# ruc-aimc-lab/GeoFormer

Measured on NVIDIA B200. Metric: pairs_per_sec_640x480, higher is better.
Workload: dtype tf32 / fp16 tensor-core operands with fp32 accumulation (fp32 residual stream, fp16 intermediates), split-fp16 similarity, f16 backbone activations

## Files before the change

geoformer_b200/_lib.py:

```python
from __future__ import annotations

import ctypes
import os
from ctypes import c_char_p, c_float, c_int, c_int64, c_void_p

HERE = os.path.dirname(os.path.abspath(__file__))
LIB_PATH = os.path.join(HERE, "libgeoformer_sm100.so")

P, I, L, F = c_void_p, c_int, c_int64, c_float

SIGNATURES = {
    "gf_abi_version": (I, []),
    "gf_last_error": (c_char_p, []),
    "gf_init": (I, [I]),
    "gf_launch_count": (L, []),
    "gf_linear_tf32": (I, [P, P, P, P, L, I, I, I, I, I, P, P, I, P, P, P, P, P]),
    "gf_linear_ref": (I, [P, P, P, P, L, I, I, I, I, I, P, P, I, P, P, P, P, P]),
    "gf_conv3x3_f16": (I, [P, P, P, P, P, I, I, I, I, I, I, I, P]),
    "gf_conv_f16": (I, [P, P, P, P, P, I, I, I, I, I, I, I, I, I, P]),
    "gf_stem_conv7x7_f16": (I, [P, P, P, P, I, I, I, P]),
    "gf_upsample_add_f16": (I, [P, P, P, I, I, I, I, I, I, P]),
    "gf_conv_ref": (I, [P, P, P, P, P, I, I, I, I, I, I, I, I, P]),
    "gf_upsample_add_ref": (I, [P, P, P, I, I, I, I, I, I, P]),
    "gf_add_posenc": (I, [P, P, P, I, L, I, P]),
    "gf_linattn_partial_floats": (L, [I, I, I, I]),
    "gf_linear_mixed": (I, [P, P, P, P, I, I, L, I, I, I, I, I, P, P, I, P, P, P, P, P]),
    "gf_fine_layer": (I, [P, P, P, P, P, P, P, P, L, P]),
    "gf_linattn_reduce_f16": (I, [P, I, P, I, I, I, I, I, P, P, P, P]),
    "gf_linattn_apply_f16": (I, [P, I, P, P, P, I, I, I, I, I, P]),
    "gf_linattn_window_f16": (I, [P, I, P, I, P, I, P, L, I, I, I, P]),
    "gf_linattn_reduce": (I, [P, I, P, I, I, I, I, I, P, P, P, P]),
    "gf_linattn_apply": (I, [P, I, P, P, P, I, I, I, I, I, P]),
    "gf_linattn_window": (I, [P, I, P, I, P, I, P, L, I, I, I, P]),
    "gf_pack_split_f16": (I, [P, P, L, I, F, I, P]),
    "gf_similarity_f16x3": (I, [P, P, P, I, I, I, I, F, P]),
    "gf_similarity_ref": (I, [P, P, P, I, I, I, I, F, F, P]),
    "gf_dual_softmax_workspace_floats": (L, [I, I, I]),
    "gf_dual_softmax_stats": (I, [P, I, I, I, P, P, P, P, P, P]),
    "gf_dual_softmax_conf": (I, [P, I, I, I, P, P, P, P, P, P, P]),
    "gf_conf_row_col_max": (I, [P, I, I, I, P, P, P]),
    "gf_mnn_select": (I, [P, I, I, I, F, I, I, I, I, I, P, P, P, P, P]),
    "gf_coarse_match_fused_workspace_bytes": (L, [I, I, I]),
    "gf_coarse_match_fused": (I, [P, P, I, I, I, I, F, F, I, I, I, I, I, P, P, P, P]),
    "gf_coarse_match_fused_pass": (I, [P, P, I, I, I, I, F, P, I, P]),
    "gf_compact_coarse": (I, [P, P, I, I, I, I, F, P, P, P, P, P, P, P, P, L, P]),
    "gf_geo_window_table": (I, [P, P, I, I, I, I, I, I, I, I, P, P]),
    "gf_geo_self_attention": (I, [P, I, P, I, P, I, P, I, I, I, I, P, P, I, P]),
    "gf_gather_anchor_kv": (I, [P, I, P, I, I, I, I, I, P, P, I, I, P, P, P]),
    "gf_gather_anchor_kv_f16": (I, [P, I, P, I, P, I, I, I, I, I, P, P, I, I, P, P, P, P]),
    "gf_geo_self_attention_tc": (I, [P, I, P, P, P, I, I, I, I, I, P, P]),
    "gf_gather_anchor_kv_h16": (I, [P, I, P, I, I, I, I, I, P, P, I, I, P, P, P]),
    "gf_masked_softmax_rows": (I, [P, I, I, I, I, P, P]),
    "gf_gemm_tf32_batched": (I, [P, L, L, P, L, L, P, L, L, I, I, I, I, F, P]),
    "gf_geo_cross_attention": (I, [P, I, P, I, P, I, P, I, I, I, I, I, P, I, P]),
    "gf_geo_cross_attention_f16": (I, [P, I, P, I, P, I, P, I, I, I, I, I, P, I, P]),
    "gf_select_rows": (I, [P, P, P, I, L, I, P]),
    "gf_fine_gather": (I, [P, I, I, I, P, P, L, I, I, I, P, P]),
    "gf_fine_gather_f16": (I, [P, I, I, I, P, P, L, I, I, I, P, P]),
    "gf_fine_gather_f16_f16": (I, [P, I, I, I, P, P, L, I, I, I, P, P]),
    "gf_gather_rows": (I, [P, L, I, P, P, L, P, P]),
    "gf_fine_match": (I, [P, P, L, I, I, F, F, P, P, P, P, P, P]),
    "gf_resize_gray_u8": (I, [P, I, I, P, I, I, P]),
    "gf_ransac_workspace_bytes": (L, [I, I]),
    "gf_ransac_homography": (I, [P, P, P, P, L, I, I, F, ctypes.c_uint, I, I, I, I, I, P, P, P, P, P, P, P, P, P, P, P, I, P]),
    "gf_compact_fine": (I, [P, P, P, P, P, P, P, L, I, F, F, F, P, P, P, P, P, P]),
    "gf_mask_rows": (I, [P, I, L, L, L, L, P, P]),
    "gf_mask_fill_sim": (I, [P, I, I, I, P, P, F, P]),
}


class GeoFormerLibError(RuntimeError):
    pass


_lib = None
_initialised_devices = set()


def load() -> ctypes.CDLL:
    global _lib
    if _lib is not None:
        return _lib
    if not os.path.exists(LIB_PATH):
        raise GeoFormerLibError(
            f"{LIB_PATH} not found - build it with `python -m geoformer_b200.build` "
            "(there is no CPU or PyTorch fallback for the hot path)")
    lib = ctypes.CDLL(LIB_PATH)
    for name, (res, args) in SIGNATURES.items():
        fn = getattr(lib, name)
        fn.restype = res
        fn.argtypes = args
    if lib.gf_abi_version() != 1:
        raise GeoFormerLibError("ABI version mismatch")
    _lib = lib
    return lib


def init(device_index: int) -> None:
    lib = load()
    if device_index in _initialised_devices:
        return
    rc = lib.gf_init(int(device_index))
    if rc != 0:
        raise GeoFormerLibError(f"gf_init({device_index}) failed: {lib.gf_last_error().decode()} (rc={rc})")
    _initialised_devices.add(device_index)


def call(name: str, *args):
    lib = load()
    rc = getattr(lib, name)(*args)
    if rc != 0:
        raise GeoFormerLibError(f"{name} failed: {lib.gf_last_error().decode()} (rc={rc})")


def launch_count() -> int:
    return int(load().gf_launch_count())
```

geoformer_b200/csrc/geo_attention.cu:

```cuda
#include "common.cuh"

#include <atomic>
#include <cuda_fp16.h>

namespace gf {
extern std::atomic<int64_t> g_launches;

__global__ void geo_window_table_kernel(const float* __restrict__ hmat, const int* __restrict__ has_h, int n, int l,
                                        int w_src_c, int h_dst_px, int w_dst_px, int w_dst_c, int scale, int window,
                                        int* __restrict__ widx) {
  const int64_t idx = (int64_t)blockIdx.x * blockDim.x + threadIdx.x;
  if (idx >= (int64_t)n * l) return;
  const int b = (int)(idx / l);
  const int tok = (int)(idx - (int64_t)b * l);
  int* out = widx + idx * window * window;
  if (!has_h[b]) {
    for (int w = 0; w < window * window; ++w) out[w] = -1;
    return;
  }
  const float* H = hmat + b * 9;
  const float x = (float)((tok % w_src_c) * scale), y = (float)((tok / w_src_c) * scale);
  float wx = __fmaf_rn(H[2], 1.f, __fmaf_rn(H[1], y, __fmul_rn(H[0], x)));
  float wy = __fmaf_rn(H[5], 1.f, __fmaf_rn(H[4], y, __fmul_rn(H[3], x)));
  float wz = __fmaf_rn(H[8], 1.f, __fmaf_rn(H[7], y, __fmul_rn(H[6], x)));
  if (wz == 0.f) wz = 1e-6f;
  const float cx = __fdiv_rn(wx, wz), cy = __fdiv_rn(wy, wz);
  const int half = window / 2;
  for (int r = 0; r < window; ++r) {
    for (int c = 0; c < window; ++c) {
      const float kx = __fadd_rn(cx, (float)((c - half) * scale));
      const float ky = __fadd_rn(cy, (float)((r - half) * scale));
      const bool oob = (kx < 0.f) | (ky < 0.f) | (kx >= (float)w_dst_px) | (ky >= (float)h_dst_px) | !(kx == kx) | !(ky == ky);
      int t = -1;
      if (!oob) t = ((int)ky / scale) * w_dst_c + ((int)kx / scale);
      out[r * window + c] = t;
    }
  }
}

constexpr int kSA = 64;
constexpr int kSAPad = kSA + 4;

__global__ void __launch_bounds__(256)
geo_self_attention_kernel(const float* __restrict__ q, int ldq, const float* __restrict__ k, int ldk,
                          const float* __restrict__ v, int ldv, float* __restrict__ out, int l, int heads,
                          const int* __restrict__ anchor_idx, const int* __restrict__ anchor_cnt, int anchor_cap,
                          float softmax_scale) {
  extern __shared__ float sh[];
  float* Qs = sh;
  float* Kt = Qs + kSA * kSA;
  float* Vs = Kt + kSA * kSAPad;
  float* Ps = Vs + kSA * kSAPad;
  const int n = blockIdx.z, h = blockIdx.y, q0 = blockIdx.x * kSA;
  const int cnt = anchor_cnt[n];
  const int c = heads * kSA;
  const int tid = threadIdx.x, tx = tid & 15, ty = tid >> 4;
  if (cnt == 0) {
    for (int e = tid; e < kSA * kSA; e += 256) {
      const int r = e >> 6, d = e & 63;
      if (q0 + r < l) out[((int64_t)n * l + q0 + r) * c + h * kSA + d] = 0.f;
    }
    return;
  }
  for (int e = tid; e < kSA * kSA; e += 256) {
    const int r = e >> 6, d = e & 63;
    Qs[e] = (q0 + r < l) ? q[((int64_t)n * l + q0 + r) * ldq + h * kSA + d] : 0.f;
  }
  float m_run[4], l_run[4], o[4][4];
#pragma unroll
  for (int i = 0; i < 4; ++i) {
    m_run[i] = -INFINITY; l_run[i] = 0.f;
#pragma unroll
    for (int j = 0; j < 4; ++j) o[i][j] = 0.f;
  }
  const int* aidx = anchor_idx + (int64_t)n * anchor_cap;
  for (int k0 = 0; k0 < cnt; k0 += kSA) {
    __syncthreads();
    for (int e = tid; e < kSA * kSA; e += 256) {
      const int r = e >> 6, d = e & 63;
      float kv = 0.f, vv = 0.f;
      if (k0 + r < cnt) {
        const int64_t tok = (int64_t)n * l + aidx[k0 + r];
        kv = k[tok * ldk + h * kSA + d];
        vv = v[tok * ldv + h * kSA + d];
      }
// ... 11 lines not shown
      const float4 kk = *reinterpret_cast<const float4*>(&Kt[d * kSAPad + 4 * tx]);
#pragma unroll
      for (int i = 0; i < 4; ++i) {
        const float qv = Qs[(4 * ty + i) * kSA + d];
        s[i][0] = fmaf(qv, kk.x, s[i][0]); s[i][1] = fmaf(qv, kk.y, s[i][1]);
        s[i][2] = fmaf(qv, kk.z, s[i][2]); s[i][3] = fmaf(qv, kk.w, s[i][3]);
      }
    }
    float alpha[4];
#pragma unroll
    for (int i = 0; i < 4; ++i) {
      float mx = -INFINITY;
#pragma unroll
      for (int j = 0; j < 4; ++j) {
        s[i][j] = (k0 + 4 * tx + j < cnt) ? s[i][j] * softmax_scale : -INFINITY;
        mx = fmaxf(mx, s[i][j]);
      }
#pragma unroll
      for (int off = 8; off > 0; off >>= 1) mx = fmaxf(mx, __shfl_xor_sync(0xffffffffu, mx, off));
      const float m_new = fmaxf(m_run[i], mx);
      alpha[i] = expf(m_run[i] - m_new);
      float rs = 0.f;
#pragma unroll
      for (int j = 0; j < 4; ++j) { s[i][j] = expf(s[i][j] - m_new); rs += s[i][j]; }
#pragma unroll
      for (int off = 8; off > 0; off >>= 1) rs += __shfl_xor_sync(0xffffffffu, rs, off);
      l_run[i] = l_run[i] * alpha[i] + rs;
      m_run[i] = m_new;
      *reinterpret_cast<float4*>(&Ps[(4 * ty + i) * kSAPad + 4 * tx]) = make_float4(s[i][0], s[i][1], s[i][2], s[i][3]);
#pragma unroll
      for (int j = 0; j < 4; ++j) o[i][j] *= alpha[i];
    }
    __syncthreads();
#pragma unroll 8
    for (int kk = 0; kk < kSA; ++kk) {
      const float4 vv = *reinterpret_cast<const float4*>(&Vs[kk * kSAPad + 4 * tx]);
#pragma unroll
      for (int i = 0; i < 4; ++i) {
        const float pv = Ps[(4 * ty + i) * kSAPad + kk];
        o[i][0] = fmaf(pv, vv.x, o[i][0]); o[i][1] = fmaf(pv, vv.y, o[i][1]);
        o[i][2] = fmaf(pv, vv.z, o[i][2]); o[i][3] = fmaf(pv, vv.w, o[i][3]);
      }
    }
  }
#pragma unroll
  for (int i = 0; i < 4; ++i) {
    const int r = q0 + 4 * ty + i;
    if (r < l) {
      const float inv = 1.f / l_run[i];
      *reinterpret_cast<float4*>(&out[((int64_t)n * l + r) * c + h * kSA + 4 * tx]) =
          make_float4(o[i][0] * inv, o[i][1] * inv, o[i][2] * inv, o[i][3] * inv);
    }
  }
}

__device__ __forceinline__ void load8(const float* p, float (&v)[8]) {
  const float4 a = *reinterpret_cast<const float4*>(p), b = *reinterpret_cast<const float4*>(p + 4);
  v[0] = a.x; v[1] = a.y; v[2] = a.z; v[3] = a.w; v[4] = b.x; v[5] = b.y; v[6] = b.z; v[7] = b.w;
}
__device__ __forceinline__ void load8(const __half* p, float (&v)[8]) {
  const uint4 u = *reinterpret_cast<const uint4*>(p);
  const uint32_t w[4] = {u.x, u.y, u.z, u.w};
#pragma unroll
  for (int i = 0; i < 4; ++i) {
    const float2 f = __half22float2(*reinterpret_cast<const __half2*>(&w[i]));
    v[2 * i] = f.x; v[2 * i + 1] = f.y;
  }
}
__device__ __forceinline__ void store8(float* p, const float (&v)[8]) {
  *reinterpret_cast<float4*>(p) = make_float4(v[0], v[1], v[2], v[3]);
  *reinterpret_cast<float4*>(p + 4) = make_float4(v[4], v[5], v[6], v[7]);
}
__device__ __forceinline__ void store8(__half* p, const float (&v)[8]) {
  uint4 u;
  __half2 h;
  h = __floats2half2_rn(v[0], v[1]); u.x = *reinterpret_cast<uint32_t*>(&h);
  h = __floats2half2_rn(v[2], v[3]); u.y = *reinterpret_cast<uint32_t*>(&h);
  h = __floats2half2_rn(v[4], v[5]); u.z = *reinterpret_cast<uint32_t*>(&h);
  h = __floats2half2_rn(v[6], v[7]); u.w = *reinterpret_cast<uint32_t*>(&h);
  *reinterpret_cast<uint4*>(p) = u;
}

template <typename T>
__global__ void geo_cross_attention_kernel(const T* __restrict__ q, int ldq, const T* __restrict__ kp, int ldk,
                                           const T* __restrict__ vp, int ldv, T* __restrict__ out, int n, int l,
                                           int s, const int* __restrict__ widx, int window2, float softmax_scale) {
  const int64_t tok = (int64_t)blockIdx.x * (blockDim.x >> 5) + (threadIdx.x >> 5);
  const int lane = threadIdx.x & 31;
  if (tok >= (int64_t)n * l) return;
  const int b = (int)(tok / l);
  const int* wi = widx + tok * window2;
  float qv[8];
  load8(q + tok * ldq + lane * 8, qv);
  float sc[25];
  int id[25];
  float mx = -INFINITY;
  int live = 0;
#pragma unroll
  for (int w = 0; w < 25; ++w) {
    const int t = w < window2 ? wi[w] : -1;
    id[w] = t;
    float d = 0.f;
    if (t >= 0) {
      float kv[8];
      load8(kp + ((int64_t)b * s + t) * ldk + lane * 8, kv);
      d = qv[0] * kv[0] + qv[1] * kv[1] + qv[2] * kv[2] + qv[3] * kv[3] + qv[4] * kv[4] + qv[5] * kv[5] + qv[6] * kv[6] + qv[7] * kv[7];
      ++live;
    }
    d += __shfl_xor_sync(0xffffffffu, d, 1);
    d += __shfl_xor_sync(0xffffffffu, d, 2);
    d += __shfl_xor_sync(0xffffffffu, d, 4);
    sc[w] = (t >= 0 ? d : -1e8f) * softmax_scale;
    if (w < window2) mx = fmaxf(mx, sc[w]);
  }
  float acc[8] = {0.f, 0.f, 0.f, 0.f, 0.f, 0.f, 0.f, 0.f};
  if (live > 0) {
    float den = 0.f;
#pragma unroll
    for (int w = 0; w < 25; ++w) {
      if (w < window2) { sc[w] = expf(sc[w] - mx); den += sc[w]; }
    }
    const float inv = 1.f / den;
#pragma unroll
    for (int w = 0; w < 25; ++w) {
      if (w < window2 && id[w] >= 0) {
        const float p = sc[w] * inv;
        float vv[8];
        load8(vp + ((int64_t)b * s + id[w]) * ldv + lane * 8, vv);
#pragma unroll
        for (int i = 0; i < 8; ++i) acc[i] = fmaf(p, vv[i], acc[i]);
      }
    }
  }
  store8(out + tok * 256 + lane * 8, acc);
}

__global__ void gather_anchor_kv_kernel(const float* __restrict__ k, int ldk, const float* __restrict__ v, int ldv,
                                        int n, int l, int heads, int dim, const int* __restrict__ anchor_idx,
                                        const int* __restrict__ anchor_cnt, int anchor_cap, int s_pad,
                                        float* __restrict__ kg, float* __restrict__ vt) {
  const int c = heads * dim;
  const int64_t idx = (int64_t)blockIdx.x * blockDim.x + threadIdx.x;
  if (idx >= (int64_t)n * s_pad * c) return;
  const int ch = (int)(idx % c);
  const int64_t r = idx / c;
  const int s = (int)(r % s_pad), b = (int)(r / s_pad);
  const int h = ch / dim, d = ch - h * dim;
  float kv = 0.f, vv = 0.f;
  if (s < anchor_cnt[b]) {
    const int64_t tok = (int64_t)b * l + anchor_idx[(int64_t)b * anchor_cap + s];
    kv = k[tok * ldk + ch];
    vv = v[tok * ldv + ch];
  }
  kg[(((int64_t)h * n + b) * s_pad + s) * dim + d] = kv;
  vt[(((int64_t)h * n + b) * dim + d) * s_pad + s] = vv;
}

__global__ void gather_anchor_kv_f16_kernel(const float* __restrict__ q, int ldq, const float* __restrict__ k, int ldk,
                                            const float* __restrict__ v, int ldv, int n, int l, int heads, int dim,
                                            const int* __restrict__ anchor_idx, const int* __restrict__ anchor_cnt,
                                            int anchor_cap, int s_pad, __half* __restrict__ q16, __half* __restrict__ kg,
                                            __half* __restrict__ vt) {
  const int c = heads * dim;
  const int64_t idx = (int64_t)blockIdx.x * blockDim.x + threadIdx.x;
  const int64_t n_kv = (int64_t)n * s_pad * c, n_q = (int64_t)n * l * c;
  if (idx < n_kv) {
    const int ch = (int)(idx % c);
    const int64_t r = idx / c;
    const int s = (int)(r % s_pad), b = (int)(r / s_pad);
    const int h = ch / dim, d = ch - h * dim;
    float kv = 0.f, vv = 0.f;
    if (s < anchor_cnt[b]) {
      const int64_t tok = (int64_t)b * l + anchor_idx[(int64_t)b * anchor_cap + s];
      kv = k[tok * ldk + ch];
      vv = v[tok * ldv + ch];
    }
    kg[(((int64_t)h * n + b) * s_pad + s) * dim + d] = __float2half_rn(kv);
    vt[(((int64_t)h * n + b) * dim + d) * s_pad + s] = __float2half_rn(vv);
  } else if (idx < n_kv + n_q) {
    const int64_t e = idx - n_kv;
    const int64_t row = e / c;
    q16[e] = __float2half_rn(q[row * ldq + (e - row * c)]);
  }
}

__global__ void __launch_bounds__(256)
gather_anchor_kv_h16_kernel(const __half* __restrict__ k, int ldk, const __half* __restrict__ v, int ldv, int n, int l,
                            const int* __restrict__ anchor_idx, const int* __restrict__ anchor_cnt, int anchor_cap,
                            int s_pad, __half* __restrict__ kg, __half* __restrict__ vt) {
  constexpr int C = 256, D = 64, PITCH = C + 8;
  __shared__ __align__(16) __half vs[64 * PITCH];
  const int b = blockIdx.y, s0 = blockIdx.x * 64, t = threadIdx.x;
  const int cnt = anchor_cnt[b];
#pragma unroll
  for (int i = 0; i < 8; ++i) {
    const int e = t + 256 * i, r = e >> 5, q = e & 31;
    const int s = s0 + r;
    uint4 kq = make_uint4(0u, 0u, 0u, 0u), vq = kq;
    if (s < cnt) {
      const int64_t tok = (int64_t)b * l + anchor_idx[(int64_t)b * anchor_cap + s];
      kq = __ldg(reinterpret_cast<const uint4*>(k + tok * ldk) + q);
      vq = __ldg(reinterpret_cast<const uint4*>(v + tok * ldv) + q);
    }
    if (s < s_pad) {
      const int h = q >> 3;
      *reinterpret_cast<uint4*>(kg + (((int64_t)h * n + b) * s_pad + s) * D + (q & 7) * 8) = kq;
    }
    *reinterpret_cast<uint4*>(vs + r * PITCH + q * 8) = vq;
  }
  __syncthreads();
  const int h = t >> 6, d = t & 63;
  __half* dst = vt + (((int64_t)h * n + b) * D + d) * s_pad + s0;
#pragma unroll
  for (int g8 = 0; g8 < 8; ++g8) {
    if (s0 + 8 * g8 >= s_pad) break;
    __half tmp[8];
#pragma unroll
// ... 18 lines not shown
    for (int i = 0; i < PER_LANE; ++i) {
      const int j = lane + 32 * i;
      v[i] = j < cnt ? p[j] : -INFINITY;
      m = fmaxf(m, v[i]);
    }
    m = warp_max(m);
    float sum = 0.f;
#pragma unroll
    for (int i = 0; i < PER_LANE; ++i) { v[i] = (lane + 32 * i < cnt) ? expf(v[i] - m) : 0.f; sum += v[i]; }
    sum = warp_sum(sum);
    const float inv = cnt > 0 ? 1.f / sum : 0.f;
#pragma unroll
    for (int i = 0; i < PER_LANE; ++i) {
      const int j = lane + 32 * i;
      if (j < s_pad) p[j] = v[i] * inv;
    }
  } else {
    float m = -INFINITY;
    for (int j = lane; j < cnt; j += 32) m = fmaxf(m, p[j]);
    m = warp_max(m);
    float sum = 0.f;
    for (int j = lane; j < cnt; j += 32) sum += expf(p[j] - m);
    sum = warp_sum(sum);
    const float inv = cnt > 0 ? 1.f / sum : 0.f;
    for (int j = lane; j < s_pad; j += 32) p[j] = j < cnt ? expf(p[j] - m) * inv : 0.f;
  }
}

}

using namespace gf;
#define STREAM ((cudaStream_t)stream)

extern "C" int gf_geo_window_table(const float* hmat, const int* has_h, int n, int h_src_c, int w_src_c, int h_dst_px,
                                   int w_dst_px, int w_dst_c, int scale, int window, int* widx, gf_stream_t stream) {
  if (n <= 0 || h_src_c <= 0 || w_src_c <= 0 || scale <= 0 || window <= 0 || window > 5)
    return gf_set_error(GF_ERR_ARG, "gf_geo_window_table: bad shape");
  const int l = h_src_c * w_src_c;
  geo_window_table_kernel<<<gf_cdiv((int64_t)n * l, 128), 128, 0, STREAM>>>(hmat, has_h, n, l, w_src_c, h_dst_px, w_dst_px,
                                                                          w_dst_c, scale, window, widx);
  g_launches++;
  GF_CHECK_LAUNCH();
  return GF_OK;
}

extern "C" int gf_geo_self_attention(const float* q, int ldq, const float* k, int ldk, const float* v, int ldv,
                                     float* out, int n, int l, int heads, int dim, const int* anchor_idx,
                                     const int* anchor_cnt, int anchor_cap, gf_stream_t stream) {
  if (n <= 0 || l <= 0 || heads <= 0 || dim != 64) return gf_set_error(GF_ERR_ARG, "gf_geo_self_attention: dim must be 64");
  const size_t smem = (size_t)(kSA * kSA + 3 * kSA * kSAPad) * sizeof(float);
  GF_SMEM_OPTIN(geo_self_attention_kernel, smem);
  geo_self_attention_kernel<<<dim3(gf_cdiv(l, kSA), heads, n), 256, smem, STREAM>>>(
      q, ldq, k, ldk, v, ldv, out, l, heads, anchor_idx, anchor_cnt, anchor_cap, 1.f / sqrtf((float)dim));
  g_launches++;
  GF_CHECK_LAUNCH();
  return GF_OK;
}

extern "C" int gf_geo_cross_attention(const float* q, int ldq, const float* kproj, int ldk, const float* vproj, int ldv,
                                      float* out, int n, int l, int s, int heads, int dim, const int* widx, int window2,
                                      gf_stream_t stream) {
  if (n <= 0 || l <= 0 || s <= 0 || heads * dim != 256 || dim != 64 || window2 <= 0 || window2 > 25)
    return gf_set_error(GF_ERR_ARG, "gf_geo_cross_attention: needs heads*dim == 256, dim == 64, window <= 25");
  geo_cross_attention_kernel<float><<<gf_cdiv((int64_t)n * l, 4), 128, 0, STREAM>>>(q, ldq, kproj, ldk, vproj, ldv, out, n, l, s,
                                                                                   widx, window2, 1.f / sqrtf((float)dim));
  g_launches++;
  GF_CHECK_LAUNCH();
  return GF_OK;
}

extern "C" int gf_geo_cross_attention_f16(const void* q, int ldq, const void* kproj, int ldk, const void* vproj, int ldv,
                                          void* out, int n, int l, int s, int heads, int dim, const int* widx, int window2,
                                          gf_stream_t stream) {
  if (n <= 0 || l <= 0 || s <= 0 || heads * dim != 256 || dim != 64 || window2 <= 0 || window2 > 25 || (ldq % 8) || (ldk % 8) || (ldv % 8))
    return gf_set_error(GF_ERR_ARG, "gf_geo_cross_attention_f16: needs heads*dim == 256, dim == 64, window <= 25, 16-byte rows");
  geo_cross_attention_kernel<__half><<<gf_cdiv((int64_t)n * l, 4), 128, 0, STREAM>>>(
      (const __half*)q, ldq, (const __half*)kproj, ldk, (const __half*)vproj, ldv, (__half*)out, n, l, s, widx, window2,
      1.f / sqrtf((float)dim));
  g_launches++;
  GF_CHECK_LAUNCH();
  return GF_OK;
}

extern "C" int gf_gather_anchor_kv(const float* k, int ldk, const float* v, int ldv, int n, int l, int heads, int dim,
                                   const int* anchor_idx, const int* anchor_cnt, int anchor_cap, int s_pad, float* kg,
                                   float* vt, gf_stream_t stream) {
  if (n <= 0 || l <= 0 || heads <= 0 || dim <= 0 || s_pad <= 0) return gf_set_error(GF_ERR_ARG, "gf_gather_anchor_kv: bad shape");
  const int64_t total = (int64_t)n * s_pad * heads * dim;
  gather_anchor_kv_kernel<<<gf_cdiv(total, 256), 256, 0, STREAM>>>(k, ldk, v, ldv, n, l, heads, dim, anchor_idx, anchor_cnt,
                                                                   anchor_cap, s_pad, kg, vt);
  g_launches++;
  GF_CHECK_LAUNCH();
  return GF_OK;
}

extern "C" int gf_gather_anchor_kv_f16(const float* q, int ldq, const float* k, int ldk, const float* v, int ldv, int n,
                                       int l, int heads, int dim, const int* anchor_idx, const int* anchor_cnt,
                                       int anchor_cap, int s_pad, void* q16, void* kg, void* vt, gf_stream_t stream) {
  if (n <= 0 || l <= 0 || heads <= 0 || dim <= 0 || s_pad <= 0) return gf_set_error(GF_ERR_ARG, "gf_gather_anchor_kv_f16: bad shape");
  const int64_t total = (int64_t)n * (s_pad + l) * heads * dim;
  gather_anchor_kv_f16_kernel<<<gf_cdiv(total, 256), 256, 0, STREAM>>>(q, ldq, k, ldk, v, ldv, n, l, heads, dim, anchor_idx,
                                                                       anchor_cnt, anchor_cap, s_pad, (__half*)q16, (__half*)kg,
                                                                       (__half*)vt);
  g_launches++;
  GF_CHECK_LAUNCH();
  return GF_OK;
}

extern "C" int gf_gather_anchor_kv_h16(const void* k, int ldk, const void* v, int ldv, int n, int l, int heads, int dim,
                                       const int* anchor_idx, const int* anchor_cnt, int anchor_cap, int s_pad, void* kg,
                                       void* vt, gf_stream_t stream) {
  if (n <= 0 || l <= 0 || heads * dim != 256 || dim != 64 || s_pad <= 0 || (s_pad % 8) || (ldk % 8) || (ldv % 8))
    return gf_set_error(GF_ERR_ARG, "gf_gather_anchor_kv_h16: needs 4 heads of dim 64, s_pad % 8 == 0, 16-byte aligned rows");
  gather_anchor_kv_h16_kernel<<<dim3(gf_cdiv(s_pad, 64), n), 256, 0, STREAM>>>((const __half*)k, ldk, (const __half*)v, ldv, n, l,
                                                                             anchor_idx, anchor_cnt, anchor_cap, s_pad,
                                                                             (__half*)kg, (__half*)vt);
  g_launches++;
  GF_CHECK_LAUNCH();
  return GF_OK;
}

extern "C" int gf_masked_softmax_rows(float* x, int heads, int n, int l, int s_pad, const int* cnt_per_sample,
                                      gf_stream_t stream) {
  if (heads <= 0 || n <= 0 || l <= 0 || s_pad <= 0) return gf_set_error(GF_ERR_ARG, "gf_masked_softmax_rows: bad shape");
  const int64_t rows = (int64_t)heads * n * l;
  if (s_pad <= 512)       masked_softmax_rows_kernel<16><<<gf_cdiv(rows, 8), 256, 0, STREAM>>>(x, rows, n, l, s_pad, cnt_per_sample);
  else if (s_pad <= 1024) masked_softmax_rows_kernel<32><<<gf_cdiv(rows, 8), 256, 0, STREAM>>>(x, rows, n, l, s_pad, cnt_per_sample);
  else if (s_pad <= 2048) masked_softmax_rows_kernel<64><<<gf_cdiv(rows, 8), 256, 0, STREAM>>>(x, rows, n, l, s_pad, cnt_per_sample);
  else                    masked_softmax_rows_kernel<0><<<gf_cdiv(rows, 8), 256, 0, STREAM>>>(x, rows, n, l, s_pad, cnt_per_sample);
  g_launches++;
  GF_CHECK_LAUNCH();
  return GF_OK;
}
```

geoformer_b200/ops.py:

```python
from __future__ import annotations

import os
import threading
from typing import Optional, Tuple

import torch

from . import _lib

EPI_RELU, EPI_TANH, EPI_ELU1, EPI_LN = 1, 2, 4, 8

_LINEAR_IMPL = "tf32"
_SIM_IMPL = "f16x3"
_ATTN_IMPL = "tf32"
_ACT16 = os.environ.get("GF_ACT16", "1") != "0"


def act16() -> bool:
    return _ACT16 and _LINEAR_IMPL == "tf32"


def set_precision(linear: Optional[str] = None, similarity: Optional[str] = None,
                  attention: Optional[str] = None, activations: Optional[str] = None) -> None:
    global _LINEAR_IMPL, _SIM_IMPL, _ATTN_IMPL, _ACT16
# ... 367 lines not shown
    _call("gf_pack_split_f16", f0.data_ptr(), a3.data_ptr(), n * l, c, in_scale, 0, _stream())
    _call("gf_pack_split_f16", f1.data_ptr(), b3.data_ptr(), n * s, c, in_scale, 1, _stream())
    ws = torch.empty(_lib.load().gf_coarse_match_fused_workspace_bytes(n, l, s), device=dev, dtype=torch.uint8)
    mj = torch.empty((n, l), device=dev, dtype=torch.int32)
    mc = torch.empty((n, l), device=dev, dtype=torch.float32)
    _call("gf_coarse_match_fused", a3.data_ptr(), b3.data_ptr(), n, l, s, 3 * c, 1.0 / temperature, float(thr), int(border),
          hw0c[0], hw0c[1], hw1c[0], hw1c[1], ws.data_ptr(), mj.data_ptr(), mc.data_ptr(), _stream())
    return _compact(mj, mc, n, l, hw0c, hw1c, scale, dev)


def mutual_nearest(conf: torch.Tensor, crmax: torch.Tensor, ccmax: torch.Tensor, thr: float, border: int,
                   hw0c: Tuple[int, int], hw1c: Tuple[int, int], scale: float):
    _chk(conf)
    n, l, s = conf.shape
    dev = conf.device
    mj = torch.empty((n, l), device=dev, dtype=torch.int32)
    mc = torch.empty((n, l), device=dev, dtype=torch.float32)
    _call("gf_mnn_select", conf.data_ptr(), n, l, s, float(thr), int(border), hw0c[0], hw0c[1], hw1c[0], hw1c[1],
              crmax.data_ptr(), ccmax.data_ptr(), mj.data_ptr(), mc.data_ptr(), _stream())
    cap = n * l
    b_ids = torch.empty(cap, device=dev, dtype=torch.int64); i_ids = torch.empty_like(b_ids); j_ids = torch.empty_like(b_ids)
    mconf = torch.empty(cap, device=dev); k0 = torch.empty((cap, 2), device=dev); k1 = torch.empty((cap, 2), device=dev)
    counts = torch.empty(n + 1, device=dev, dtype=torch.int32)
    _call("gf_compact_coarse", mj.data_ptr(), mc.data_ptr(), n, l, hw0c[1], hw1c[1], float(scale), b_ids.data_ptr(),
              i_ids.data_ptr(), j_ids.data_ptr(), mconf.data_ptr(), k0.data_ptr(), k1.data_ptr(), counts.data_ptr(),
              counts.data_ptr() + 4 * n, cap, _stream())
    counts_h = counts.cpu()
    total = int(counts_h[n])
    return dict(b_ids=b_ids[:total], i_ids=i_ids[:total], j_ids=j_ids[:total], m_bids=b_ids[:total],
                mconf=mconf[:total], mkpts0_c=k0[:total], mkpts1_c=k1[:total]), counts_h[:n]


def geo_window_table(hmat: torch.Tensor, has_h: torch.Tensor, n: int, hw_src_c, hw_dst_px, w_dst_c: int, scale: int,
                     window: int) -> torch.Tensor:
    l = hw_src_c[0] * hw_src_c[1]
    widx = torch.empty((n, l, window * window), device=hmat.device, dtype=torch.int32)
    _call("gf_geo_window_table", hmat.data_ptr(), has_h.data_ptr(), n, hw_src_c[0], hw_src_c[1], hw_dst_px[0],
              hw_dst_px[1], w_dst_c, scale, window, widx.data_ptr(), _stream())
    return widx


def geo_self_attention(q, ldq, k, ldk, v, ldv, n, l, heads, dim, anchor_idx, anchor_cnt, max_cnt: int = 0,
                       impl: Optional[str] = None) -> torch.Tensor:
    c = heads * dim
    out = torch.empty((n * l, c), device=q.device, dtype=torch.float32)
    mode = impl or _ATTN_IMPL
    if mode in ("tf32", "tf32_mat") and max_cnt > 0:
        s_pad = (max_cnt + 63) // 64 * 64
        dev = q.device
        if mode == "tf32":
            kg = torch.empty((heads, n, s_pad, dim), device=dev, dtype=torch.float16)
            vt = torch.empty((heads, n, dim, s_pad), device=dev, dtype=torch.float16)
            if q.dtype == torch.float16:
                _call("gf_gather_anchor_kv_h16", k.data_ptr(), ldk, v.data_ptr(), ldv, n, l, heads, dim,
                      anchor_idx.data_ptr(), anchor_cnt.data_ptr(), anchor_idx.shape[1], s_pad, kg.data_ptr(),
                      vt.data_ptr(), _stream())
                q16, ld16 = q, ldq
            else:
                q16, ld16 = torch.empty((n * l, c), device=dev, dtype=torch.float16), c
                _call("gf_gather_anchor_kv_f16", q.data_ptr(), ldq, k.data_ptr(), ldk, v.data_ptr(), ldv, n, l, heads, dim,
                      anchor_idx.data_ptr(), anchor_cnt.data_ptr(), anchor_idx.shape[1], s_pad, q16.data_ptr(),
                      kg.data_ptr(), vt.data_ptr(), _stream())
            _call("gf_geo_self_attention_tc", q16.data_ptr(), ld16, kg.data_ptr(), vt.data_ptr(), out.data_ptr(), n, l,
                  heads, dim, s_pad, anchor_cnt.data_ptr(), _stream())
            return out
        kg = torch.empty((heads, n, s_pad, dim), device=dev, dtype=torch.float32)
        vt = torch.empty((heads, n, dim, s_pad), device=dev, dtype=torch.float32)
        _call("gf_gather_anchor_kv", k.data_ptr(), ldk, v.data_ptr(), ldv, n, l, heads, dim, anchor_idx.data_ptr(),
              anchor_cnt.data_ptr(), anchor_idx.shape[1], s_pad, kg.data_ptr(), vt.data_ptr(), _stream())
        sc = torch.empty((heads, n, l, s_pad), device=dev, dtype=torch.float32)
        for h in range(heads):
            _call("gf_gemm_tf32_batched", q.data_ptr() + 4 * h * dim, ldq, l * ldq, kg[h].data_ptr(), dim, s_pad * dim,
                  sc[h].data_ptr(), s_pad, l * s_pad, l, s_pad, dim, n, 1.0 / dim ** 0.5, _stream(), tag="[QK]")
        _call("gf_masked_softmax_rows", sc.data_ptr(), heads, n, l, s_pad, anchor_cnt.data_ptr(), _stream())
        for h in range(heads):
            _call("gf_gemm_tf32_batched", sc[h].data_ptr(), s_pad, l * s_pad, vt[h].data_ptr(), s_pad, dim * s_pad,
                  out.data_ptr() + 4 * h * dim, c, l * c, l, dim, s_pad, n, 1.0, _stream(), tag="[PV]")
        return out
    _call("gf_geo_self_attention", q.data_ptr(), ldq, k.data_ptr(), ldk, v.data_ptr(), ldv, out.data_ptr(), n, l,
              heads, dim, anchor_idx.data_ptr(), anchor_cnt.data_ptr(), anchor_idx.shape[1], _stream())
    return out


def geo_cross_attention(q, ldq, kp, ldk, vp, ldv, n, l, s, heads, dim, widx) -> torch.Tensor:
    out = torch.empty((n * l, heads * dim), device=q.device, dtype=q.dtype)
    _call("gf_geo_cross_attention" + ("_f16" if q.dtype == torch.float16 else ""), q.data_ptr(), ldq, kp.data_ptr(), ldk, vp.data_ptr(), ldv, out.data_ptr(), n,
              l, s, heads, dim, widx.data_ptr(), widx.shape[2], _stream())
    return out


def select_rows_(dst: torch.Tensor, src: torch.Tensor, flag: torch.Tensor, n: int, l: int, c: int) -> None:
    _call("gf_select_rows", dst.data_ptr(), src.data_ptr(), flag.data_ptr(), n, l, c, _stream())


def fine_gather(fine_nhwc: torch.Tensor, b_ids, tok_ids, wc: int, stride: int, window: int,
                out: Optional[torch.Tensor] = None) -> torch.Tensor:
    _, hf, wf, c = fine_nhwc.shape
    assert fine_nhwc.is_contiguous()
    m = b_ids.shape[0]
    if out is None:
        out = torch.empty((m, window * window, c), device=fine_nhwc.device, dtype=torch.float32)
    if out.dtype == torch.float16:
        assert fine_nhwc.dtype == torch.float16
        fn = "gf_fine_gather_f16_f16"
    else:
        fn = "gf_fine_gather_f16" if fine_nhwc.dtype == torch.float16 else "gf_fine_gather"
    _call(fn, fine_nhwc.data_ptr(), hf, wf, c, b_ids.data_ptr(), tok_ids.data_ptr(), m, wc, stride,
              window, out.data_ptr(), _stream())
    return out


def gather_rows(feat: torch.Tensor, b_ids, tok_ids, out: Optional[torch.Tensor] = None) -> torch.Tensor:
    _, l, c = feat.shape
    assert feat.is_contiguous()
    m = b_ids.shape[0]
    if out is None:
        out = torch.empty((m, c), device=feat.device, dtype=torch.float32)
    _call("gf_gather_rows", feat.data_ptr(), l, c, b_ids.data_ptr(), tok_ids.data_ptr(), m, out.data_ptr(), _stream())
    return out


def fine_match(f0: torch.Tensor, f1: torch.Tensor, temperature: float, thr: float, mkpts0_c, mkpts1_c, b_ids,
               window: int, coarse_scale: float, c2f: float, fine_scale: float, want_matrix: bool = False):
    m, ww, c = f0.shape
    dev = f0.device
    sel = torch.empty(m, device=dev, dtype=torch.int32); fi = torch.empty_like(sel); fj = torch.empty_like(sel)
    fconf = torch.empty(m, device=dev)
    fmat = torch.empty((m, ww, ww), device=dev) if want_matrix else None
    _call("gf_fine_match", f0.data_ptr(), f1.data_ptr(), m, ww, c, float(temperature), float(thr), sel.data_ptr(),
              fi.data_ptr(), fj.data_ptr(), fconf.data_ptr(), _ptr(fmat), _stream())
    k0 = torch.empty((m, 2), device=dev); k1 = torch.empty((m, 2), device=dev); mconf = torch.empty(m, device=dev)
    mb = torch.empty(m, device=dev, dtype=torch.int64); total = torch.empty(1, device=dev, dtype=torch.int32)
    _call("gf_compact_fine", sel.data_ptr(), fi.data_ptr(), fj.data_ptr(), fconf.data_ptr(), mkpts0_c.data_ptr(),
              mkpts1_c.data_ptr(), b_ids.data_ptr(), m, window, float(coarse_scale), float(c2f), float(fine_scale),
              k0.data_ptr(), k1.data_ptr(), mconf.data_ptr(), mb.data_ptr(), total.data_ptr(), _stream())
    t = int(total.item())
    return dict(mkpts0_f=k0[:t], mkpts1_f=k1[:t], mconf=mconf[:t], m_bids=mb[:t]), fmat, (sel, fi, fj, fconf)


def ransac_homography(k0: torch.Tensor, k1: torch.Tensor, b_ids: torch.Tensor, counts: torch.Tensor, n: int,
                      hw0_c, hw1_c, scale: int, thr: float = 8.0, hyps: int = 1024, seed: int = 0):
    dev = k0.device
    _chk(k0); _chk(k1); _chk(b_ids, torch.int64); _chk(counts, torch.int32)
    assert k0.is_contiguous() and k1.is_contiguous()
    m = int(k0.shape[0])
    l0, l1 = hw0_c[0] * hw0_c[1], hw1_c[0] * hw1_c[1]
    cap = max(l0, l1)
    ws = torch.empty(_lib.load().gf_ransac_workspace_bytes(n, hyps), device=dev, dtype=torch.uint8)
    hm = torch.empty((2, n, 9), device=dev)
    has_h = torch.empty(n, device=dev, dtype=torch.int32)
    inlier = torch.empty(max(m, 1), device=dev, dtype=torch.int32)
    map0 = torch.empty((n, l0), device=dev, dtype=torch.int32); map1 = torch.empty((n, l1), device=dev, dtype=torch.int32)
    aidx = torch.zeros((2, n, cap), device=dev, dtype=torch.int32)
    acnt = torch.empty((2, n), device=dev, dtype=torch.int32)
    _call("gf_ransac_homography", k0.data_ptr(), k1.data_ptr(), b_ids.data_ptr(), counts.data_ptr(), m, n, hyps,
          float(thr), int(seed) & 0xffffffff, int(scale), l0, hw0_c[1], l1, hw1_c[1], ws.data_ptr(), hm[0].data_ptr(),
          hm[1].data_ptr(), has_h.data_ptr(), inlier.data_ptr(), map0.data_ptr(), map1.data_ptr(), aidx[0].data_ptr(),
          acnt[0].data_ptr(), aidx[1].data_ptr(), acnt[1].data_ptr(), cap, _stream(), tag="ransac")
    return hm, has_h, inlier[:m], aidx, acnt


def resize_gray_u8(src: torch.Tensor, dst: torch.Tensor) -> torch.Tensor:
    if not src.is_cuda or not dst.is_cuda:
        raise _lib.GeoFormerLibError("geoformer_b200 ops need CUDA tensors (no CPU fallback)")
    assert src.dtype == torch.uint8 and src.dim() == 2 and src.is_contiguous()
    assert dst.dtype == torch.float32 and dst.dim() == 2 and dst.is_contiguous()
    _call("gf_resize_gray_u8", src.data_ptr(), src.shape[0], src.shape[1], dst.data_ptr(), dst.shape[0], dst.shape[1], _stream())
    return dst
# ... 1 lines not shown
```

include/geoformer_b200.h:

```cpp
#ifndef GEOFORMER_B200_H_
#define GEOFORMER_B200_H_

#include <stdint.h>

#ifdef __cplusplus
extern "C" {
#endif

#define GF_ABI_VERSION 1

#define GF_OK 0
#define GF_ERR_ARG (-1)
#define GF_ERR_LAUNCH (-2)
#define GF_ERR_DRIVER (-3)
#define GF_ERR_DEVICE (-4)

#define GF_EPI_RELU 1
#define GF_EPI_TANH 2
#define GF_EPI_ELU1 4
#define GF_EPI_LN 8

typedef void* gf_stream_t;

int gf_abi_version(void);
// ... 15 lines not shown

int gf_conv3x3_f16(const void* x, const void* wt, const float* bias, const void* residual, void* y, int batch, int h,
                    int w, int cin_p, int cout_p, int cin_k, int act, gf_stream_t stream);
int gf_conv_f16(const void* x, const void* wt, const float* bias, const void* residual, void* y, int batch, int h, int w,
                 int cin_p, int cout_p, int cin_k, int ksize, int stride, int act, gf_stream_t stream);

int gf_stem_conv7x7_f16(const float* img, const float* wperm, const float* bias, void* out, int batch, int h, int w,
                         gf_stream_t stream);
int gf_upsample_add_f16(const void* lateral, const void* src, void* out, int batch, int h, int w, int hs, int ws,
                         int c, gf_stream_t stream);
int gf_conv_ref(const float* x, const float* wt, const float* bias, const float* residual, float* y, int batch, int h,
                int w, int cin, int cout, int ksize, int stride, int act, gf_stream_t stream);
int gf_upsample_add_ref(const float* lateral, const float* src, float* out, int batch, int h, int w, int hs, int ws,
                        int c, gf_stream_t stream);

int gf_add_posenc(const float* x, const float* pe, float* out, int n, int64_t l, int c, gf_stream_t stream);

int64_t gf_linattn_partial_floats(int n, int s, int heads, int dim);
int gf_linattn_reduce(const float* K, int ldk, const float* V, int ldv, int n, int s, int heads, int dim,
                      float* partial, float* KV, float* Ksum, gf_stream_t stream);
int gf_linattn_apply(const float* Q, int ldq, const float* KV, const float* Ksum, float* out, int n, int l, int s,
                     int heads, int dim, gf_stream_t stream);
int gf_linattn_window(const float* Q, int ldq, const float* K, int ldk, const float* V, int ldv, float* out,
                      int64_t n_windows, int tokens, int heads, int dim, gf_stream_t stream);
int gf_linattn_reduce_f16(const void* K, int ldk, const void* V, int ldv, int n, int s, int heads, int dim,
                          float* partial, float* KV, float* Ksum, gf_stream_t stream);
int gf_linattn_apply_f16(const void* Q, int ldq, const float* KV, const float* Ksum, void* out, int n, int l, int s,
                         int heads, int dim, gf_stream_t stream);
int gf_linattn_window_f16(const void* Q, int ldq, const void* K, int ldk, const void* V, int ldv, void* out,
                          int64_t n_windows, int tokens, int heads, int dim, gf_stream_t stream);

int gf_pack_split_f16(const float* x, void* out_f16, int64_t rows, int c, float scale, int role, gf_stream_t stream);
int gf_similarity_f16x3(const void* a3, const void* b3, float* sim, int n, int l, int s, int c3, float out_scale,
                        gf_stream_t stream);
int gf_similarity_ref(const float* f0, const float* f1, float* sim, int n, int l, int s, int c, float in_scale,
                      float out_scale, gf_stream_t stream);
int64_t gf_dual_softmax_workspace_floats(int n, int l, int s);
int gf_dual_softmax_stats(const float* sim, int n, int l, int s, float* row_max, float* row_sum, float* col_max,
                          float* col_sum, float* workspace, gf_stream_t stream);
int gf_dual_softmax_conf(float* sim_conf, int n, int l, int s, const float* row_max, const float* row_sum,
                         const float* col_max, const float* col_sum, float* conf_row_max, float* conf_col_max,
                         gf_stream_t stream);
int gf_conf_row_col_max(const float* conf, int n, int l, int s, float* conf_row_max, float* conf_col_max,
                        gf_stream_t stream);
int gf_mnn_select(const float* conf, int n, int l, int s, float thr, int border, int h0c, int w0c, int h1c, int w1c,
                  const float* conf_row_max, const float* conf_col_max, int* match_j, float* match_conf,
                  gf_stream_t stream);
int64_t gf_coarse_match_fused_workspace_bytes(int n, int l, int s);
int gf_coarse_match_fused(const void* a3, const void* b3, int n, int l, int s, int c3, float out_scale, float thr,
                          int border, int h0c, int w0c, int h1c, int w1c, void* workspace, int* match_j,
                          float* match_conf, gf_stream_t stream);
int gf_coarse_match_fused_pass(const void* a3, const void* b3, int n, int l, int s, int c3, float out_scale,
                               void* workspace, int pass, gf_stream_t stream);
int gf_compact_coarse(const int* match_j, const float* match_conf, int n, int l, int w0c, int w1c, float scale,
                      int64_t* b_ids, int64_t* i_ids, int64_t* j_ids, float* mconf, float* mkpts0_c, float* mkpts1_c,
                      int* counts, int* total, int64_t capacity, gf_stream_t stream);

int gf_geo_window_table(const float* hmat, const int* has_h, int n, int h_src_c, int w_src_c, int h_dst_px, int w_dst_px,
                        int w_dst_c, int scale, int window, int* widx, gf_stream_t stream);
int gf_geo_self_attention(const float* q, int ldq, const float* k, int ldk, const float* v, int ldv, float* out,
                          int n, int l, int heads, int dim, const int* anchor_idx, const int* anchor_cnt,
                          int anchor_cap, gf_stream_t stream);
int gf_gather_anchor_kv(const float* k, int ldk, const float* v, int ldv, int n, int l, int heads, int dim,
                        const int* anchor_idx, const int* anchor_cnt, int anchor_cap, int s_pad, float* kg, float* vt,
                        gf_stream_t stream);
int gf_masked_softmax_rows(float* x, int heads, int n, int l, int s_pad, const int* cnt_per_sample, gf_stream_t stream);
int gf_gather_anchor_kv_f16(const float* q, int ldq, const float* k, int ldk, const float* v, int ldv, int n, int l,
                            int heads, int dim, const int* anchor_idx, const int* anchor_cnt, int anchor_cap, int s_pad,
                            void* q16, void* kg, void* vt, gf_stream_t stream);
int gf_gather_anchor_kv_h16(const void* k, int ldk, const void* v, int ldv, int n, int l, int heads, int dim,
                            const int* anchor_idx, const int* anchor_cnt, int anchor_cap, int s_pad, void* kg, void* vt,
                            gf_stream_t stream);
int gf_geo_self_attention_tc(const void* q16, int ldq, const void* kg, const void* vt, float* out, int n, int l,
                             int heads, int dim, int s_pad, const int* anchor_cnt, gf_stream_t stream);
int gf_gemm_tf32_batched(const float* A, int64_t lda, int64_t a_batch_stride, const float* B, int64_t ldb,
                         int64_t b_batch_stride, float* Y, int64_t ldy, int64_t y_batch_stride, int M, int N, int K,
                         int batches, float out_scale, gf_stream_t stream);

int gf_geo_cross_attention(const float* q, int ldq, const float* kproj, int ldk, const float* vproj, int ldv,
                           float* out, int n, int l, int s, int heads, int dim, const int* widx, int window2,
                           gf_stream_t stream);
int gf_geo_cross_attention_f16(const void* q, int ldq, const void* kproj, int ldk, const void* vproj, int ldv, void* out,
                               int n, int l, int s, int heads, int dim, const int* widx, int window2, gf_stream_t stream);
int gf_select_rows(float* dst, const float* src, const int* flag, int n, int64_t l, int c, gf_stream_t stream);

int gf_fine_layer(const float* x, const float* src, const void* wpack, const float* gamma1, const float* beta1,
                  const float* gamma2, const float* beta2, float* y, int64_t windows, gf_stream_t stream);
int gf_fine_gather(const float* fine_nhwc, int hf, int wf, int c, const int64_t* b_ids, const int64_t* tok_ids,
                   int64_t m, int wc, int stride, int window, float* out, gf_stream_t stream);
int gf_fine_gather_f16(const void* fine_nhwc, int hf, int wf, int c, const int64_t* b_ids, const int64_t* tok_ids,
                        int64_t m, int wc, int stride, int window, float* out, gf_stream_t stream);
int gf_fine_gather_f16_f16(const void* fine_nhwc, int hf, int wf, int c, const int64_t* b_ids, const int64_t* tok_ids,
                            int64_t m, int wc, int stride, int window, void* out, gf_stream_t stream);
int gf_gather_rows(const float* feat, int64_t l, int c, const int64_t* b_ids, const int64_t* tok_ids, int64_t m,
                   float* out, gf_stream_t stream);
int gf_fine_match(const float* f0, const float* f1, int64_t m, int ww, int c, float temperature, float thr,
                  int* sel, int* fi, int* fj, float* fconf, float* fine_matrix, gf_stream_t stream);
int gf_compact_fine(const int* sel, const int* fi, const int* fj, const float* fconf, const float* mkpts0_c,
                    const float* mkpts1_c, const int64_t* b_ids, int64_t m, int window, float coarse_scale,
                    float c2f_scale, float fine_scale, float* mkpts0_f, float* mkpts1_f, float* mconf,
                    int64_t* m_bids, int* total, gf_stream_t stream);

int gf_resize_gray_u8(const void* src, int ho, int wo, float* dst, int ht, int wt, gf_stream_t stream);

int64_t gf_ransac_workspace_bytes(int n, int hyps);
int gf_ransac_homography(const float* k0, const float* k1, const int64_t* b_ids, const int* counts, int64_t m, int n,
                         int hyps, float thr, unsigned seed, int scale, int l0, int w0c, int l1, int w1c,
                         void* workspace, float* hmat, float* hinv, int* has_h, int* inlier, int* map0, int* map1,
                         int* anchor_idx0, int* anchor_cnt0, int* anchor_idx1, int* anchor_cnt1, int cap,
                         gf_stream_t stream);

int gf_mask_rows(void* buf, int elem_bytes, int64_t rows, int64_t ld, int64_t col0, int64_t cols, const uint8_t* mask,
                 gf_stream_t stream);
int gf_mask_fill_sim(float* sim, int n, int l, int s, const uint8_t* mask0, const uint8_t* mask1, float fill,
                     gf_stream_t stream);

#ifdef __cplusplus
}
#endif
#endif
```

Baseline: 469.5.

## Tile geo cross-attention queries and stage deduplicated K/V rows in shared memory

Adds a tiled fp16 cross-attention kernel. Each block handles 32 queries for one head, builds a bitmap of the unique key tokens their windows reference, compacts them, and copies those K/V rows into shared memory with cp.async, so overlapping windows reuse staged rows instead of issuing repeated global loads. If the referenced rows span too wide or exceed the capacity, the tile falls back to global loads. The fp16 path now uses this kernel by default, at the cost of extra setup work (atomics, prefix scan, several barriers) per tile.

```diff
diff --git a/geoformer_b200/_lib.py b/geoformer_b200/_lib.py
--- a/geoformer_b200/_lib.py
+++ b/geoformer_b200/_lib.py
@@ -54,6 +54,7 @@
     "gf_gemm_tf32_batched": (I, [P, L, L, P, L, L, P, L, L, I, I, I, I, F, P]),
     "gf_geo_cross_attention": (I, [P, I, P, I, P, I, P, I, I, I, I, I, P, I, P]),
     "gf_geo_cross_attention_f16": (I, [P, I, P, I, P, I, P, I, I, I, I, I, P, I, P]),
+    "gf_geo_cross_attention_f16_tiles": (I, [P, I, P, I, P, I, P, I, I, I, I, I, P, I, P, P]),
     "gf_select_rows": (I, [P, P, P, I, L, I, P]),
     "gf_fine_gather": (I, [P, I, I, I, P, P, L, I, I, I, P, P]),
     "gf_fine_gather_f16": (I, [P, I, I, I, P, P, L, I, I, I, P, P]),
diff --git a/geoformer_b200/csrc/geo_attention.cu b/geoformer_b200/csrc/geo_attention.cu
--- a/geoformer_b200/csrc/geo_attention.cu
+++ b/geoformer_b200/csrc/geo_attention.cu
@@ -1,6 +1,7 @@
 #include "common.cuh"
 
 #include <atomic>
+#include <climits>
 #include <cuda_fp16.h>
 
 namespace gf {
@@ -178,6 +179,72 @@
 }
 
 template <typename T>
+struct GlobalRows {
+  const T* k;
+  const T* v;
+  int64_t ldk, ldv;
+  static constexpr bool kAlwaysLoad = false;
+  __device__ const T* krow(int t) const { return k + t * ldk; }
+  __device__ const T* vrow(int t) const { return v + t * ldv; }
+};
+struct SharedRows {
+  const __half* k;
+  const __half* v;
+  int zero;
+  static constexpr bool kAlwaysLoad = true;
+  __device__ const __half* krow(int t) const { return k + (t < 0 ? zero : t) * 64; }
+  __device__ const __half* vrow(int t) const { return v + (t < 0 ? zero : t) * 64; }
+};
+
+template <typename T, class Rows>
+__device__ __forceinline__ void cross_attend_query(const T* qp, const int* wi, bool valid, int window2, float softmax_scale,
+                                                   const Rows& rows, float (&acc)[8]) {
+  float qv[8] = {0.f, 0.f, 0.f, 0.f, 0.f, 0.f, 0.f, 0.f};
+  if (valid) load8(qp, qv);
+  float sc[25];
+  int id[25];
+  float mx = -INFINITY;
+  int live = 0;
+#pragma unroll
+  for (int w = 0; w < 25; ++w) {
+    const int t = (valid && w < window2) ? wi[w] : -1;
+    id[w] = t;
+    float d = 0.f;
+    if (Rows::kAlwaysLoad || t >= 0) {
+      float kv[8];
+      load8(rows.krow(t), kv);
+      d = qv[0] * kv[0] + qv[1] * kv[1] + qv[2] * kv[2] + qv[3] * kv[3] + qv[4] * kv[4] + qv[5] * kv[5] + qv[6] * kv[6] + qv[7] * kv[7];
+    }
+    live += t >= 0;
+    d += __shfl_xor_sync(0xffffffffu, d, 1);
+    d += __shfl_xor_sync(0xffffffffu, d, 2);
+    d += __shfl_xor_sync(0xffffffffu, d, 4);
+    sc[w] = (t >= 0 ? d : -1e8f) * softmax_scale;
+    if (w < window2) mx = fmaxf(mx, sc[w]);
+  }
+#pragma unroll
+  for (int i = 0; i < 8; ++i) acc[i] = 0.f;
+  if (live > 0) {
+    float den = 0.f;
+#pragma unroll
+    for (int w = 0; w < 25; ++w) {
+      if (w < window2) { sc[w] = expf(sc[w] - mx); den += sc[w]; }
+    }
+    const float inv = 1.f / den;
+#pragma unroll
+    for (int w = 0; w < 25; ++w) {
+      if (w < window2 && (Rows::kAlwaysLoad || id[w] >= 0)) {
+        const float p = sc[w] * inv;
+        float vv[8];
+        load8(rows.vrow(id[w]), vv);
+#pragma unroll
+        for (int i = 0; i < 8; ++i) acc[i] = fmaf(p, vv[i], acc[i]);
+      }
+    }
+  }
+}
+
+template <typename T>
 __global__ void geo_cross_attention_kernel(const T* __restrict__ q, int ldq, const T* __restrict__ kp, int ldk,
                                            const T* __restrict__ vp, int ldv, T* __restrict__ out, int n, int l,
                                            int s, const int* __restrict__ widx, int window2, float softmax_scale) {
@@ -185,50 +252,118 @@
   const int lane = threadIdx.x & 31;
   if (tok >= (int64_t)n * l) return;
   const int b = (int)(tok / l);
-  const int* wi = widx + tok * window2;
-  float qv[8];
-  load8(q + tok * ldq + lane * 8, qv);
-  float sc[25];
-  int id[25];
-  float mx = -INFINITY;
-  int live = 0;
-#pragma unroll
-  for (int w = 0; w < 25; ++w) {
-    const int t = w < window2 ? wi[w] : -1;
-    id[w] = t;
-    float d = 0.f;
+  const GlobalRows<T> rows{kp + (int64_t)b * s * ldk + lane * 8, vp + (int64_t)b * s * ldv + lane * 8, ldk, ldv};
+  float acc[8];
+  cross_attend_query(q + tok * ldq + lane * 8, widx + tok * window2, true, window2, softmax_scale, rows, acc);
+  store8(out + tok * 256 + lane * 8, acc);
+}
+
+constexpr int kXQ = 32;
+constexpr int kXThreads = kXQ * 8;
+constexpr int kXCap = 256;
+constexpr int kXSpan = 2048;
+constexpr size_t kXSmem = (size_t)2 * (kXCap + 1) * 64 * sizeof(__half) + (size_t)kXQ * 25 * sizeof(int) + kXCap * sizeof(int) +
+                          (kXSpan / 32) * 2 * sizeof(uint32_t) + 16;
+
+__device__ __forceinline__ void cp_async16(void* smem, const void* gmem) {
+  const uint32_t sa = (uint32_t)__cvta_generic_to_shared(smem);
+  asm volatile("cp.async.cg.shared.global [%0], [%1], 16;" ::"r"(sa), "l"(gmem));
+}
+
+__global__ void __launch_bounds__(kXThreads, 3)
+geo_cross_attention_tiles_kernel(const __half* __restrict__ q, int ldq, const __half* __restrict__ kp, int ldk,
+                                 const __half* __restrict__ vp, int ldv, __half* __restrict__ out, int l, int s,
+                                 const int* __restrict__ widx, int window2, float softmax_scale, int* __restrict__ fallback_tiles) {
+  constexpr int kWords = kXSpan / 32;
+  extern __shared__ __align__(16) unsigned char xsm[];
+  __half* ks = reinterpret_cast<__half*>(xsm);
+  __half* vs = ks + (kXCap + 1) * 64;
+  int* slot = reinterpret_cast<int*>(vs + (kXCap + 1) * 64);
+  int* row_tok = slot + kXQ * 25;
+  uint32_t* bits = reinterpret_cast<uint32_t*>(row_tok + kXCap);
+  uint32_t* below = bits + kWords;
+  int* info = reinterpret_cast<int*>(below + kWords);
+
+  const int tid = threadIdx.x, g = tid >> 3, j = tid & 7;
+  const int h = blockIdx.y, b = blockIdx.z, q0 = blockIdx.x * kXQ;
+  const int nq = min(kXQ, l - q0);
+  const int ne = nq * window2;
+  const int* wt = widx + ((int64_t)b * l + q0) * window2;
+  if (tid < kWords) bits[tid] = 0u;
+  if (tid < 16) reinterpret_cast<uint4*>(tid < 8 ? ks + kXCap * 64 : vs + kXCap * 64)[tid & 7] = make_uint4(0u, 0u, 0u, 0u);
+  if (tid == 0) { info[0] = INT_MAX; info[2] = 0; }
+  __syncthreads();
+  int tmin = INT_MAX;
+  for (int e = tid; e < ne; e += kXThreads) {
+    const int t = __ldg(wt + e);
+    slot[e] = t;
+    if (t >= 0) tmin = min(tmin, t);
+  }
+  tmin = __reduce_min_sync(0xffffffffu, tmin);
+  if ((tid & 31) == 0 && tmin != INT_MAX) atomicMin(&info[0], tmin);
+  __syncthreads();
+  tmin = info[0];
+  for (int e = tid; e < ne; e += kXThreads) {
+    const int t = slot[e];
     if (t >= 0) {
-      float kv[8];
-      load8(kp + ((int64_t)b * s + t) * ldk + lane * 8, kv);
-      d = qv[0] * kv[0] + qv[1] * kv[1] + qv[2] * kv[2] + qv[3] * kv[3] + qv[4] * kv[4] + qv[5] * kv[5] + qv[6] * kv[6] + qv[7] * kv[7];
-      ++live;
-    }
-    d += __shfl_xor_sync(0xffffffffu, d, 1);
-    d += __shfl_xor_sync(0xffffffffu, d, 2);
-    d += __shfl_xor_sync(0xffffffffu, d, 4);
-    sc[w] = (t >= 0 ? d : -1e8f) * softmax_scale;
-    if (w < window2) mx = fmaxf(mx, sc[w]);
-  }
-  float acc[8] = {0.f, 0.f, 0.f, 0.f, 0.f, 0.f, 0.f, 0.f};
-  if (live > 0) {
-    float den = 0.f;
-#pragma unroll
-    for (int w = 0; w < 25; ++w) {
-      if (w < window2) { sc[w] = expf(sc[w] - mx); den += sc[w]; }
-    }
-    const float inv = 1.f / den;
-#pragma unroll
-    for (int w = 0; w < 25; ++w) {
-      if (w < window2 && id[w] >= 0) {
-        const float p = sc[w] * inv;
-        float vv[8];
-        load8(vp + ((int64_t)b * s + id[w]) * ldv + lane * 8, vv);
-#pragma unroll
-        for (int i = 0; i < 8; ++i) acc[i] = fmaf(p, vv[i], acc[i]);
+      const int o = t - tmin;
+      if (o < kXSpan) atomicOr(&bits[o >> 5], 1u << (o & 31));
+      else info[2] = 1;
+    }
+  }
+  __syncthreads();
+  if (tid < 32) {
+    const int c0 = __popc(bits[2 * tid]), c1 = __popc(bits[2 * tid + 1]);
+    int x = c0 + c1;
+#pragma unroll
+    for (int off = 1; off < 32; off <<= 1) {
+      const int y = __shfl_up_sync(0xffffffffu, x, off);
+      if (tid >= off) x += y;
+    }
+    below[2 * tid] = x - c0 - c1;
+    below[2 * tid + 1] = x - c1;
+    if (tid == 31) info[1] = x;
+  }
+  __syncthreads();
+  const int rows = info[1];
+  const bool valid = g < nq;
+  const int64_t tok = (int64_t)b * l + q0 + g;
+  const __half* qp = q + tok * ldq + h * 64 + j * 8;
+  float acc[8];
+  if (info[2] || rows > kXCap) {
+    if (tid == 0 && fallback_tiles) atomicAdd(fallback_tiles, 1);
+    const GlobalRows<__half> gr{kp + (int64_t)b * s * ldk + h * 64 + j * 8, vp + (int64_t)b * s * ldv + h * 64 + j * 8, ldk, ldv};
+    cross_attend_query(qp, wt + g * window2, valid, window2, softmax_scale, gr, acc);
+  } else {
+    if (tid < kWords) {
+      uint32_t m = bits[tid];
+      int r = below[tid];
+      while (m) {
+        row_tok[r++] = tmin + 32 * tid + __ffs(m) - 1;
+        m &= m - 1;
       }
     }
-  }
-  store8(out + tok * 256 + lane * 8, acc);
+    __syncthreads();
+    for (int e = tid; e < rows * 16; e += kXThreads) {
+      const int r = e >> 4, c = e & 15;
+      const int64_t src = (int64_t)b * s + row_tok[r];
+      if (c < 8) cp_async16(ks + r * 64 + c * 8, kp + src * ldk + h * 64 + c * 8);
+      else       cp_async16(vs + r * 64 + (c - 8) * 8, vp + src * ldv + h * 64 + (c - 8) * 8);
+    }
+    asm volatile("cp.async.commit_group;" ::: "memory");
+    for (int e = tid; e < ne; e += kXThreads) {
+      const int t = slot[e];
+      if (t >= 0) {
+        const int o = t - tmin;
+        slot[e] = below[o >> 5] + __popc(bits[o >> 5] & ((1u << (o & 31)) - 1u));
+      }
+    }
+    asm volatile("cp.async.wait_group 0;" ::: "memory");
+    __syncthreads();
+    const SharedRows sr{ks + j * 8, vs + j * 8, kXCap};
+    cross_attend_query(qp, slot + g * window2, valid, window2, softmax_scale, sr, acc);
+  }
+  if (valid) store8(out + tok * 256 + h * 64 + j * 8, acc);
 }
 
 __global__ void gather_anchor_kv_kernel(const float* __restrict__ k, int ldk, const float* __restrict__ v, int ldv,
@@ -413,6 +548,21 @@
   return GF_OK;
 }
 
+extern "C" int gf_geo_cross_attention_f16_tiles(const void* q, int ldq, const void* kproj, int ldk, const void* vproj, int ldv,
+                                                void* out, int n, int l, int s, int heads, int dim, const int* widx,
+                                                int window2, int* fallback_tiles, gf_stream_t stream) {
+  if (n <= 0 || l <= 0 || s <= 0 || heads * dim != 256 || dim != 64 || window2 <= 0 || window2 > 25 || (ldq % 8) || (ldk % 8) || (ldv % 8))
+    return gf_set_error(GF_ERR_ARG, "gf_geo_cross_attention_f16_tiles: needs heads*dim == 256, dim == 64, window <= 25, 16-byte rows");
+  if (n > 65535) return gf_set_error(GF_ERR_ARG, "gf_geo_cross_attention_f16_tiles: n > 65535");
+  GF_SMEM_OPTIN(geo_cross_attention_tiles_kernel, kXSmem);
+  geo_cross_attention_tiles_kernel<<<dim3(gf_cdiv(l, kXQ), heads, n), kXThreads, kXSmem, STREAM>>>(
+      (const __half*)q, ldq, (const __half*)kproj, ldk, (const __half*)vproj, ldv, (__half*)out, l, s, widx, window2,
+      1.f / sqrtf((float)dim), fallback_tiles);
+  g_launches++;
+  GF_CHECK_LAUNCH();
+  return GF_OK;
+}
+
 extern "C" int gf_gather_anchor_kv(const float* k, int ldk, const float* v, int ldv, int n, int l, int heads, int dim,
                                    const int* anchor_idx, const int* anchor_cnt, int anchor_cap, int s_pad, float* kg,
                                    float* vt, gf_stream_t stream) {
diff --git a/geoformer_b200/ops.py b/geoformer_b200/ops.py
--- a/geoformer_b200/ops.py
+++ b/geoformer_b200/ops.py
@@ -473,8 +473,14 @@
     return out
 
 
-def geo_cross_attention(q, ldq, kp, ldk, vp, ldv, n, l, s, heads, dim, widx) -> torch.Tensor:
+def geo_cross_attention(q, ldq, kp, ldk, vp, ldv, n, l, s, heads, dim, widx, tiles: bool = True,
+                        fallback_tiles: Optional[torch.Tensor] = None) -> torch.Tensor:
     out = torch.empty((n * l, heads * dim), device=q.device, dtype=q.dtype)
+    if q.dtype == torch.float16 and tiles:
+        _call("gf_geo_cross_attention_f16_tiles", q.data_ptr(), ldq, kp.data_ptr(), ldk, vp.data_ptr(), ldv, out.data_ptr(),
+              n, l, s, heads, dim, widx.data_ptr(), widx.shape[2],
+              None if fallback_tiles is None else fallback_tiles.data_ptr(), _stream())
+        return out
     _call("gf_geo_cross_attention" + ("_f16" if q.dtype == torch.float16 else ""), q.data_ptr(), ldq, kp.data_ptr(), ldk, vp.data_ptr(), ldv, out.data_ptr(), n,
               l, s, heads, dim, widx.data_ptr(), widx.shape[2], _stream())
     return out
diff --git a/include/geoformer_b200.h b/include/geoformer_b200.h
--- a/include/geoformer_b200.h
+++ b/include/geoformer_b200.h
@@ -121,6 +121,9 @@
                            gf_stream_t stream);
 int gf_geo_cross_attention_f16(const void* q, int ldq, const void* kproj, int ldk, const void* vproj, int ldv, void* out,
                                int n, int l, int s, int heads, int dim, const int* widx, int window2, gf_stream_t stream);
+int gf_geo_cross_attention_f16_tiles(const void* q, int ldq, const void* kproj, int ldk, const void* vproj, int ldv,
+                                     void* out, int n, int l, int s, int heads, int dim, const int* widx, int window2,
+                                     int* fallback_tiles, gf_stream_t stream);
 int gf_select_rows(float* dst, const float* src, const int* flag, int n, int64_t l, int c, gf_stream_t stream);
 
 int gf_fine_layer(const float* x, const float* src, const void* wpack, const float* gamma1, const float* beta1,
```

Result: no change. 473.8, median of 6 (+0.9%).
